# pyranha-labs/hypergrep

Measured on AMD Instinct MI355X. Metric: GiB/s scanned (256 patterns, 32 GiB synthetic log per GPU, text resident in HBM), higher is better.
Workload: dtype u8

## Files before the change

### hypergrep_amd/build.py

```python
from __future__ import annotations

import os
import shutil
import subprocess
import sys

PKG = os.path.dirname(os.path.abspath(__file__))
REPO = os.path.dirname(PKG)
CSRC = os.path.join(PKG, "csrc")
LIB_DIR = os.path.join(PKG, "lib")
LIB = os.path.join(LIB_DIR, "libhyperscanner.so")
LIBHS_NAME = "libhs.so.5"
OBJ = os.path.join(REPO, "build", "obj")
EXTRA = os.environ.get("HG_BUILD_DEFINES", "").split()
if os.environ.get("HG_BUILD_OUT"):
    LIB = os.path.abspath(os.environ["HG_BUILD_OUT"])
    LIB_DIR = os.path.dirname(LIB)
    OBJ = LIB + ".obj"
    LIBHS_NAME = os.path.basename(LIB) + ".libhs.so.5"

HIP_SOURCES = ["hg_stream.hip", "hg_kernels.hip", "hg_always_on.hip", "hg_huge.hip", "hg_som.hip", "hg_comb.hip", "hg_invert.hip", "hg_context.hip", "hg_parts.hip", "hg_segments.hip", "hg_segctx.hip", "hg_segparts.hip", "hg_gather.hip", "hg_counts.hip", "hg_flows.hip", "hg_batch.hip", "hg_engine.hip", "hg_capi.hip", "hg_shim.hip", "hg_hsface.hip"]
CXX_SOURCES = ["hg_compile.cpp"]
HEADERS = ["hg_mem.h", "hg_db.h", "hg_core.h", "hg_post.h", "hg_engine.h", "hg_compile.h", "hg_synth.h", "hg_confirm_dev.h", "hg_sink_dev.h", "hg_tables_dev.h", "hg_som.h", "hg_comb.h", "hg_invert.h", "hg_context.h", "hg_parts.h", "hg_parts_dev.h", "hg_segments.h", "hg_segctx.h", "hg_segparts.h", "hg_gather.h", "hg_counts.h", "hg_wave_dev.h", "hg_flows.h", "hg_flow_rules.h", "hg_batch.h", "hg_batch_launch.h"]


def _hipcc() -> str:
    for cand in (shutil.which("hipcc"), "/opt/rocm/bin/hipcc"):
        if cand and os.path.exists(cand):
            return cand
    raise RuntimeError("hipcc not found: the native library can only be built with the ROCm toolchain")


def _stale(target: str, deps: list[str]) -> bool:
    if not os.path.exists(target):
        return True
    t = os.path.getmtime(target)
    return any(os.path.getmtime(d) > t for d in deps if os.path.exists(d))

# ... 120 lines not shown
```

### hypergrep_amd/csrc/hg_engine.h

```cpp
#pragma once
#include <hip/hip_runtime.h>

#include <memory>
#include <string>
#include <vector>

#include "../../include/hypergrep_amd.h"
#include "hg_compile.h"
#include "hg_core.h"
#include "hg_invert.h"
#include "hg_context.h"
#include "hg_segments.h"
#include "hg_segctx.h"
#include "hg_parts.h"
#include "hg_segparts.h"
#include "hg_gather.h"
#include "hg_counts.h"
#include "hg_mem.h"
#include "hg_post.h"

#ifndef HG_STREAM_WG_WAVES
#define HG_STREAM_WG_WAVES 8
#endif
constexpr uint32_t HG_STREAM_WG_WAVES_DEFAULT = HG_STREAM_WG_WAVES;

constexpr uint32_t HG_CONFIRM_SPLIT = 4;
constexpr uint32_t HG_DEFER_SHARDS = 64;

struct HgDeferred {
  uint64_t pos;
  uint32_t pattern;
  uint32_t rank;
};
enum { HG_ST_MINLEN_KEPT = 16, HG_ST_FIN_TOTAL = 24, HG_ST_SELECTED = 28, HG_ST_FINAL = 32, HG_ST_WORDS = 36, HG_ST_ZERO_WORDS = 32,
       HG_ST_BLOCK_DONE = 40 };
enum { HG_CNT_CANDS = 0, HG_CNT_HITS = 1, HG_CNT_CAND_NEED = 2, HG_CNT_HIT_NEED = 3, HG_CNT_DEFER_NEED = 4,
       HG_CNT_HITS_WRAPPED = 5,
       HG_CNT_JOIN_TILES = 6,
       HG_CNT_WORDS = 8,
       HG_CNT_CURSOR0 = 64,
       HG_CNT_CURSORS = 64,
       HG_ST_ALLOC_WORDS = 128 };
constexpr uint32_t HG_STREAM_GRAB = 2 * HG_STREAM_WG_WAVES_DEFAULT;

constexpr uint32_t HG_FIN_MAX_BUCKETS = 1u << 22;
constexpr uint32_t HG_FIN_BUCKET_CAP = 4096;
constexpr uint32_t HG_FIN_MEDIUM_CAP = 512;

#ifndef HG_CONFIRM_THREADS
// ... 229 lines not shown
  template <typename T>
  using DevBuf = hgmem::Buf<T, hgmem::Space::Dev>;
  int device_;
  std::vector<uint32_t> ids_host_;
  hipEvent_t ev_[2] = {nullptr, nullptr};
  DevBuf<uint32_t> ids_{"counts ids", 0}, seg_lines_{"counts seg lines", 0}, seg_reports_{"counts seg reports", 0};
  DevBuf<unsigned long long> totals_{"counts totals", 0};
};

struct HgEngineKnobs {
  uint64_t fin_target = 48;
  bool no_bucket_finalize = false;
  uint64_t chunk_tiles = 0;
  uint32_t max_chunks = 0;
  std::vector<double> chunk_weights;
  long stream_wgs_per_cu = 0;
  long joiner = -1;
  bool joiner_ahead = false;
  bool no_early_finalize = false;
  uint32_t confirm_mode_mask = 0x1F;
  long confirm_blocks_per_cu = 0;
  uint64_t hit_limit = 0;
  uint64_t cand_limit = 0;
  bool verbose = false;
  static HgEngineKnobs from_env();
};

class HgScanner {
 public:
  static int create(std::shared_ptr<const HgDb> db, int device, HgScanner **out, std::string *err);
// ... 81 lines not shown
  uint64_t chunk_limit_tiles_ = 0;
  uint32_t defer_spread_boost_ = 1;
  bool hit_direct_ = false;
  HgTileSum *d_sums_ = nullptr;
  HgTileBase *d_bases_ = nullptr, *d_block_base_ = nullptr, *d_final_ = nullptr;
  HgTileElem *d_agg_ = nullptr;
  HgCand *d_cands_ = nullptr;
  HgDeferred *d_deferred_ = nullptr;
  uint32_t *d_defer_count_ = nullptr;
  HgHit *d_hits_raw_ = nullptr, *d_hits_out_ = nullptr;
  HgHitAux *d_aux_raw_ = nullptr, *d_aux_out_ = nullptr;
  HgHit *d_acc_hits_ = nullptr;
  HgHitAux *d_acc_aux_ = nullptr;
  uint64_t acc_cap_ = 0;
  bool side_bound_ = false;
  uint64_t *d_key_a_ = nullptr, *d_key_b_ = nullptr;
  uint32_t *d_perm_a_ = nullptr, *d_perm_b_ = nullptr;
  uint8_t *d_keep_ = nullptr;
  uint32_t *d_counters_ = nullptr, *d_selected_ = nullptr, *d_seg_count_ = nullptr;
  uint32_t max_segs_ = 0;
  uint32_t *d_pflags_ = nullptr;
  void *d_temp_ = nullptr;
  size_t temp_bytes_ = 0;
  uint32_t *h_counters_ = nullptr;
  HgTileBase *h_final_ = nullptr;
  hipEvent_t ev_[4] = {nullptr, nullptr, nullptr, nullptr};
  static constexpr int kMaxChunks = 64;
  hipStream_t side_stream_ = nullptr;
  hipEvent_t ev_tile_done_ = nullptr;
  hipEvent_t ev_fin_early_ = nullptr;
  hipEvent_t ev_k1_begin_[kMaxChunks] = {}, ev_k1_end_[kMaxChunks] = {}, ev_side_done_[kMaxChunks] = {};
  uint32_t *d_fin_fill_ = nullptr, *d_fin_kept_ = nullptr, *d_fin_total_ = nullptr, *d_fin_big_ = nullptr;
  bool fin_fallback_ = false;
  uint32_t fin_alloc_ = 0;
  uint32_t fin_epoch_ = 0;
  FinInfo fin_info_{};
  uint64_t fin_expect_hits_ = 0;
  void *d_huge_claim_ = nullptr;
  uint64_t huge_claim_slots_ = 0;
  uint32_t *d_from_ = nullptr;
  uint64_t from_cap_ = 0;
  uint32_t som_max_nw_ = 0;
  uint32_t *d_min_lengths_ = nullptr;
  HgHit *d_minlen_hits_ = nullptr;
  HgHitAux *d_minlen_aux_ = nullptr;
  uint64_t minlen_cap_ = 0;
  uint32_t minlen_max_nw_ = 0;
  HgComb *d_combs_ = nullptr;
  uint32_t *d_comb_words_ = nullptr, *d_comb_feed_ = nullptr;
// ... 57 lines not shown
```

### hypergrep_amd/csrc/hg_engine.hip

```cpp
#include <algorithm>
#include <array>
#include <cstdio>
#include <cstdlib>
#include <cstring>
#include <memory>

#include "hg_engine.h"
#include "hg_mem.h"

#include <rocprim/rocprim.hpp>

bool hg_launch_stream(const HgStreamArgs &a, uint32_t grid, hipStream_t stream);
bool hg_launch_stream_join(const HgStreamArgs &a, uint32_t grid, hipStream_t stream);
int hg_stream_blocks_per_cu(uint32_t filter_log2, uint32_t filter_wide, uint32_t dense);
__global__ void hg_tile_reduce_kernel(const HgTileSum *sums, uint64_t tile_begin, uint64_t tile_end, uint64_t bs1, HgTileElem *agg);
__global__ void hg_tile_spine_kernel(const HgTileElem *agg, uint32_t nblocks, uint64_t bs1, HgTileBase *block_base, HgTileBase *state);
__global__ void hg_tile_apply_kernel(const HgTileSum *sums, uint64_t tile_begin, uint64_t tile_end, uint64_t bs1, const HgTileBase *block_base,
                                     HgTileBase *bases);
__global__ void hg_tile_inner_kernel(const uint8_t *text, HgTileSum *sums, uint64_t tile_begin, uint64_t tile_end, uint64_t bs1);
__global__ void hg_verify_kernel(HgConfirmArgs a);
__global__ void hg_confirm_fast_kernel(HgConfirmArgs a, uint32_t blocks_per_mode);
__global__ void hg_confirm_generic_kernel(HgConfirmArgs a);
__global__ void hg_always_on_kernel(HgConfirmArgs a, uint32_t first, uint32_t last);
__global__ void hg_always_on_fast_kernel(HgConfirmArgs a);
// ... 20 lines not shown
__global__ void hg_offset_kernel(uint32_t *idx, uint32_t n, uint32_t add);
__global__ void hg_key_packed_kernel(const HgHit *hits, const HgHitAux *aux, const HgPattern *patterns, uint32_t n, uint32_t id_bits, uint32_t to_bits,
                                     uint64_t *key, uint32_t *idx);
__global__ void hg_keep_kernel(const HgHit *hits, const HgHitAux *aux, const uint32_t *perm, const HgPattern *patterns, uint32_t n, uint8_t *keep);
__global__ void hg_scatter_kernel(const HgHit *hits, const HgHitAux *aux, const uint32_t *perm, const uint8_t *keep, const uint32_t *pos, uint32_t n,
                                  HgHit *oh, HgHitAux *oa, uint32_t *count);

size_t hg_huge_lds_bytes(uint32_t nw_max, uint32_t stage_cap);
bool hg_launch_confirm_huge(const HgConfirmArgs &a, uint32_t grid, uint32_t nw_max, uint32_t stage_cap, void *claim, uint32_t claim_mask, hipStream_t stream);
bool hg_launch_always_on_huge(const HgConfirmArgs &a, uint32_t grid, uint32_t nw_max, uint32_t stage_cap, uint32_t first, uint32_t last, hipStream_t stream);
bool hg_launch_block_huge(const HgConfirmArgs &a, uint32_t grid, uint32_t nw_max, uint32_t stage_cap, const uint32_t *pattern_flags, hipStream_t stream);

namespace {
constexpr int TS_BLOCK_TILES = 1024;
constexpr int STREAM_WG_WAVES = HG_STREAM_WG_WAVES;

template <typename T>
hipError_t upload(void **dst, const std::vector<T> &src, const char *name) {
  size_t bytes = std::max<size_t>(src.size() * sizeof(T), 16);
  hipError_t e = hgmem::dev_alloc(dst, bytes, name);
  if (e != hipSuccess) return e;
  if (!src.empty()) e = hipMemcpy(*dst, src.data(), src.size() * sizeof(T), hipMemcpyHostToDevice);
  return e;
}
template <typename T>
hipError_t realloc_dev(T *&ptr, size_t count, const char *name) {
  hgmem::dev_free(ptr, name);
  ptr = nullptr;
  return hgmem::dev_alloc(&ptr, std::max<size_t>(count * sizeof(T), 16), name);
}
// ... 15 lines not shown
    return env ? std::strtoull(env, nullptr, 10) : dflt;
  };
  k.fin_target = std::max<uint64_t>(4, num("HG_FIN_TARGET", 48));
  k.no_bucket_finalize = std::getenv("HG_NO_BUCKET_FINALIZE") != nullptr;
  k.chunk_tiles = num("HG_CHUNK_TILES", 0);
  k.max_chunks = static_cast<uint32_t>(std::min<uint64_t>(num("HG_MAX_CHUNKS", 0), 1u << 20));
  if (const char *env = std::getenv("HG_CHUNK_WEIGHTS")) {
    for (const char *q = env; *q;) {
      char *e = nullptr;
      const double v = std::strtod(q, &e);
      if (e == q) break;
      if (v > 0) k.chunk_weights.push_back(v);
      q = *e ? e + 1 : e;
    }
  }
  k.stream_wgs_per_cu = static_cast<long>(num("HG_STREAM_WGS_PER_CU", 0));
  if (const char *env = std::getenv("HG_JOINER")) k.joiner = std::max(0l, std::min(2l, std::strtol(env, nullptr, 10)));
  k.joiner_ahead = std::getenv("HG_JOINER_AHEAD") != nullptr;
  k.no_early_finalize = std::getenv("HG_NO_EARLY_FINALIZE") != nullptr;
#ifdef HG_PROFILE_CONFIRM
  if (const char *env = std::getenv("HG_DEBUG_CONFIRM_MODES")) k.confirm_mode_mask = static_cast<uint32_t>(std::strtoul(env, nullptr, 0));
#endif
  k.confirm_blocks_per_cu = static_cast<long>(std::min<uint64_t>(num("HG_CONFIRM_BLOCKS_PER_CU", 0), 16));
  k.hit_limit = num("HG_HIT_LIMIT", 0);
  k.cand_limit = num("HG_CAND_LIMIT", 0);
  k.verbose = std::getenv("HG_VERBOSE") != nullptr;
  return k;
}

bool HgScanner::fail(hipError_t e, const char *what) {
// ... 107 lines not shown
                  d_key_a_, d_key_b_, d_perm_a_, d_perm_b_, d_keep_, d_counters_, d_temp_, d_seg_count_, d_pflags_, d_deferred_, d_defer_count_, d_seg_count2_, d_cands2_, d_disc_, d_bucket2_, d_windows2_, d_groups_, d_acc_hits_, d_acc_aux_, d_huge_claim_, d_wtab_, d_from_, d_fin_fill_, d_fin_kept_, d_fin_big_,
                  d_combs_, d_comb_words_, d_comb_feed_, d_comb_count_, d_comb_pos_, d_comb_hits_, d_comb_aux_, d_comb_temp_, d_bounds_,
                  d_min_lengths_, d_minlen_hits_, d_minlen_aux_, d_inv_count_, d_inv_pos_, d_inv_temp_, d_inv_hits_, d_inv_aux_,
                  d_ctx_count_, d_ctx_pos_, d_ctx_temp_, d_ctx_hits_, d_ctx_aux_,
                  d_parts_first_, d_parts_count_, d_parts_pos_, d_parts_temp_, d_parts_, d_part_pattern_,
                  d_segw_, d_seg_flag_, d_seg_temp_, d_seg_hits_, d_seg_aux_, d_seg_of_, d_seg_from_, d_pad_keep_, d_pad_pos_,
                  d_segctx_first_, d_segctx_k_, d_segctx_win_, d_segctx_of_, d_segparts_first_, d_segparts_of_};
  for (void *p : ptrs) hgmem::dev_free(p, "scanner");
  hgmem::host_free(h_counters_, "h_counters_");
  for (auto &ev : ev_)
    if (ev) (void)hipEventDestroy(ev);
  for (int i = 0; i < kMaxChunks; i++) {
    if (ev_k1_begin_[i]) (void)hipEventDestroy(ev_k1_begin_[i]);
    if (ev_k1_end_[i]) (void)hipEventDestroy(ev_k1_end_[i]);
    if (ev_side_done_[i]) (void)hipEventDestroy(ev_side_done_[i]);
  }
  if (side_stream_) (void)hipStreamDestroy(side_stream_);
  if (ev_fin_early_) (void)hipEventDestroy(ev_fin_early_);
  if (ev_tile_done_) (void)hipEventDestroy(ev_tile_done_);
}

int HgScanner::alloc_cands(uint64_t n) {
  n = std::min<uint64_t>(n, 0x7FFFFFF0u);
  HG_TRY(realloc_dev(d_cands_, n, "d_cands_"), "workspace alloc (candidates)");
  HG_TRY(realloc_dev(d_cands2_, n, "d_cands2_"), "workspace alloc (candidates)");
  uint32_t modes = 0;
  for (uint32_t m = 0; m < HG_CONFIRM_MODES; m++) modes += db_->n_confirm_mode[m] ? 1 : 0;
  HG_TRY(realloc_dev(d_deferred_, std::max<uint64_t>(modes, 1) * n, "d_deferred_"), "workspace alloc (deferred)");
  hgmem::dev_free(d_huge_claim_, "d_huge_claim_");
  d_huge_claim_ = nullptr;
  huge_claim_slots_ = 0;
  if (db_->n_confirm_mode[4]) {
// ... 26 lines not shown
    temp_bytes_ = need;
  }
  return HG_OK;
}

int HgScanner::ensure(uint64_t nbytes) {
  uint64_t ntiles = std::max<uint64_t>((nbytes + HG_TILE_BYTES - 1) / HG_TILE_BYTES, 1);
  auto re = [&](auto *&ptr, size_t count, const char *name) { return fail(realloc_dev(ptr, count, name), "workspace alloc"); };
  if (ntiles > cap_tiles_) {
    uint64_t nblocks = (ntiles + TS_BLOCK_TILES - 1) / TS_BLOCK_TILES;
    if (re(d_sums_, ntiles, "d_sums_") || re(d_bases_, ntiles + 1, "d_bases_") || re(d_agg_, nblocks, "d_agg_") || re(d_block_base_, nblocks, "d_block_base_")) return HG_ERR_HIP;
    cap_tiles_ = ntiles;
  }
  if (!d_seg_count_) {
    max_segs_ = static_cast<uint32_t>(num_cus_) * 16;
    if (re(d_seg_count_, max_segs_, "d_seg_count_") || re(d_seg_count2_, max_segs_, "d_seg_count2_") || re(d_defer_count_, HG_CONFIRM_MODES * HG_DEFER_SHARDS, "d_defer_count_")) return HG_ERR_HIP;
  }
  uint64_t want = std::max<uint64_t>(nbytes / 1024, 1u << 16);
  if (cand_cap_ < want && alloc_cands(want)) return HG_ERR_HIP;
  if (hit_cap_ < want && alloc_hits(want)) return HG_ERR_HIP;
  return HG_OK;
}

enum { HG_SPLIT = 1000, HG_GROWN = 1001 };

struct HgScanner::PassPlan {
  const uint8_t *text;
  uint64_t nbytes, bs1, ntiles;
  PassRange range;
  bool block_mode, has_anchored;
  hipStream_t stream, side;
  uint32_t id_bits, to_bits, fin_shift = 10, fin_nb = 1, fin_cap;
  bool bucketed;
  uint32_t nchunks = 1;
  bool piped, split;
  uint64_t chunk_tiles;
  std::array<uint64_t, kMaxChunks + 1> cut;
  uint32_t wgs_alone, wgs_shared, joiner_wgs, wgs = 1;
  uint32_t cand_seg_cap[2];
  HgStreamArgs sa;
  HgConfirmArgs ca;
  uint32_t fin_done, stage_blocks = 1;
  uint32_t wgs_of(uint32_t c) const { return c == 0 ? wgs_alone : wgs_shared; }
  uint32_t joiners_of(uint32_t c) const { return c >= 1 ? joiner_wgs : 0u; }
  uint32_t set_of(uint32_t c) const { return piped ? (c & 1u) : 0u; }
  uint32_t settled_buckets(uint32_t c) const {
    const uint64_t prev_end = std::min<uint64_t>(cut[c] << HG_TILE_SHIFT, nbytes);
    const uint64_t settled = prev_end > bs1 ? prev_end - bs1 : 0;
    return static_cast<uint32_t>(std::min<uint64_t>((settled > range.own_lo ? settled - range.own_lo : 0) >> fin_shift, fin_nb));
  }
};

HgScanner::PassPlan HgScanner::plan_pass(const uint8_t *text, uint64_t nbytes, uint64_t bs1, uint64_t line_base, const PassRange &range, bool block_mode,
                                         hipStream_t stream) const {
  const uint64_t tile_lo = range.tile_lo, tile_hi = range.tile_hi, ntiles = tile_hi - tile_lo;
  PassPlan p{text, nbytes, bs1, ntiles, range, block_mode, db_->patterns.size() - db_->ncomb > db_->slow.size(), stream};
  const uint64_t own_end = std::min<uint64_t>(range.own_hi, nbytes), own_len = own_end > range.own_lo ? own_end - range.own_lo : 0;
// ... 29 lines not shown
  if (p.split) return p;
  for (uint32_t c = 0; c <= nchunks; c++) p.cut[c] = std::min<uint64_t>(tile_lo + static_cast<uint64_t>(c) * chunk_tiles, tile_hi);
  const std::vector<double> &w = knobs_.chunk_weights;
  if (!block_mode && w.size() >= 2 && w.size() <= static_cast<size_t>(kMaxChunks) && ntiles >= w.size() * TS_BLOCK_TILES * 2) {
    double total = 0, run = 0;
    for (double v : w) total += v;
    nchunks = static_cast<uint32_t>(w.size());
    chunk_tiles = 0;
    for (uint32_t c = 0; c < nchunks; c++) {
      run += w[c];
      uint64_t end = c + 1 == nchunks ? tile_hi : tile_lo + static_cast<uint64_t>(static_cast<double>(ntiles) * run / total) / TS_BLOCK_TILES * TS_BLOCK_TILES;
      end = std::min<uint64_t>(std::max<uint64_t>(end, p.cut[c] + TS_BLOCK_TILES), tile_hi);
      p.cut[c + 1] = end;
      chunk_tiles = std::max<uint64_t>(chunk_tiles, end - p.cut[c]);
    }
  }
  p.nchunks = nchunks;
  p.chunk_tiles = chunk_tiles;
  p.piped = nchunks > 1;
  p.side = p.piped ? side_stream_ : stream;

  if (ntiles) {
    uint32_t per_cu = p.piped ? std::max(1, stream_wgs_per_cu_ - 1) : stream_wgs_per_cu_;
    if (knobs_.stream_wgs_per_cu) {
      const long v = knobs_.stream_wgs_per_cu;
      if (v >= 1 && v <= stream_wgs_per_cu_) per_cu = static_cast<uint32_t>(v);
    }
    auto grid_for = [&](uint32_t wgs_per_cu) {
      return static_cast<uint32_t>(std::min<uint64_t>((std::min<uint64_t>(chunk_tiles, ntiles) + STREAM_WG_WAVES - 1) / STREAM_WG_WAVES,
                                                      std::min<uint64_t>(static_cast<uint64_t>(num_cus_) * wgs_per_cu, max_segs_)));
    };
    p.wgs_shared = grid_for(per_cu);
    p.wgs_alone = knobs_.stream_wgs_per_cu ? p.wgs_shared : grid_for(static_cast<uint32_t>(stream_wgs_per_cu_));
    p.joiner_wgs = (p.piped && stream_wgs_per_cu_ >= 3 && per_cu < static_cast<uint32_t>(stream_wgs_per_cu_) && chunk_limit_tiles_ == 0 && !side_bound_) ? static_cast<uint32_t>(num_cus_) : 0u;
    if (knobs_.joiner >= 0) p.joiner_wgs = p.piped ? static_cast<uint32_t>(knobs_.joiner) * static_cast<uint32_t>(num_cus_) : 0u;
// ... 51 lines not shown
int HgScanner::alloc_fin(uint32_t nb, hipStream_t stream) {
  uint32_t want = 1u << 16;
  while (want < nb) want <<= 1;
  fin_alloc_ = 0;
  HG_TRY(realloc_dev(d_fin_fill_, want, "d_fin_fill_"), "alloc finalize buckets");
  HG_TRY(realloc_dev(d_fin_kept_, want, "d_fin_kept_"), "alloc finalize buckets");
  HG_TRY(realloc_dev(d_fin_big_, 2 * static_cast<size_t>(want) + 3 * 128, "d_fin_big_"), "alloc finalize buckets");
  HG_TRY(hipMemsetAsync(d_fin_big_ + 2 * static_cast<size_t>(want), 0, 3 * 128 * 4, stream), "clear scan flags");
  fin_alloc_ = want;
  return HG_OK;
}

int HgScanner::launch_fin(const PassPlan &p, hipStream_t s, uint32_t lo, uint32_t hi, bool beside_stream) {
  if (hi <= lo) return HG_OK;
  const uint32_t nbk = hi - lo, cu = static_cast<uint32_t>(num_cus_), fin_cap = p.fin_cap, id_bits = p.id_bits, to_bits = p.to_bits;
  HG_TRY(hipMemsetAsync(d_fin_total_ + 2, 0, 8, s), "memset work list");
  hipLaunchKernelGGL(hg_fin_sort_small_kernel, dim3(std::min<uint32_t>((nbk + 3) / 4, cu * 8)), dim3(256), 0, s, d_hits_raw_, d_perm_a_, d_fin_fill_, lo, hi, fin_cap, id_bits, to_bits,
                     d_fin_kept_, d_fin_big_, d_fin_total_ + 2, fin_alloc_);
  hipLaunchKernelGGL((hg_fin_sort_big_kernel<HG_FIN_MEDIUM_CAP, true>), dim3(std::min<uint32_t>(nbk, cu * 4)), dim3(256), 0, s, d_hits_raw_, d_perm_a_, d_fin_fill_, d_fin_big_, d_fin_total_ + 2,
                     fin_cap, id_bits, to_bits, d_fin_kept_, d_selected_ + 1, static_cast<uint64_t *>(nullptr), static_cast<uint32_t *>(nullptr));
  const uint32_t big_blocks = std::min<uint32_t>(std::min<uint32_t>(nbk, 64u), hit_cap_ / HG_FIN_BUCKET_CAP);
  if (big_blocks)
    hipLaunchKernelGGL((hg_fin_sort_big_kernel<HG_FIN_BUCKET_CAP, false>), dim3(big_blocks), dim3(256), 0, s, d_hits_raw_, d_perm_a_, d_fin_fill_, d_fin_big_ + fin_alloc_,
                       d_fin_total_ + 3, fin_cap, id_bits, to_bits, d_fin_kept_, d_selected_ + 1, d_key_a_, d_perm_b_);
  const uint32_t scan_blocks = std::max<uint32_t>(1, std::min<uint32_t>(128, (nbk + 8191) / 8192));
  fin_info_.scan_blocks = std::max(fin_info_.scan_blocks, scan_blocks);
  uint32_t *part = d_fin_big_ + 2 * static_cast<size_t>(fin_alloc_);
  const uint32_t epoch = ++fin_epoch_ ? fin_epoch_ : ++fin_epoch_;
  if (beside_stream) hipLaunchKernelGGL(hg_fin_scan_kernel<512u>, dim3(scan_blocks), dim3(512), 0, s, d_fin_kept_, lo, hi, d_fin_total_, d_fin_fill_, fin_cap, part, epoch);
  else hipLaunchKernelGGL(hg_fin_scan_kernel<1024u>, dim3(scan_blocks), dim3(1024), 0, s, d_fin_kept_, lo, hi, d_fin_total_, d_fin_fill_, fin_cap, part, epoch);
  hipLaunchKernelGGL(hg_fin_gather_kernel, dim3(std::min<uint32_t>((nbk + 3) / 4, cu * 8)), dim3(256), 0, s, d_hits_raw_, d_aux_raw_, d_perm_a_, d_fin_kept_, d_fin_total_, lo, hi, fin_cap,
                     d_hits_out_, d_aux_out_);
  HG_TRY(hipGetLastError(), "finalize launch");
  return HG_OK;
}

int HgScanner::copy_fin_fill(uint32_t *dst, uint32_t max, uint32_t *n) {
  *n = 0;
  if (fin_info_.path != 1u || !d_fin_fill_ || !dst) return HG_OK;
// ... 28 lines not shown
  HG_TRY(hipEventRecord(p.piped ? ev_k1_begin_[c] : ev_[1], p.stream), "event");
  if (joiners_c && knobs_.joiner_ahead)
    if (int rc = launch_joiner(p.stream)) return rc;
  if (!hg_launch_stream(sa, wgs_c, p.stream)) return error(HG_ERR_ARG, "no stream kernel for this database's filter size / mode");
  HG_TRY(hipGetLastError(), "hg_stream_kernel launch");
  HG_TRY(hipEventRecord(p.piped ? ev_k1_end_[c] : ev_[2], p.stream), "event");
  if (p.piped && p.bucketed && joiners_c && c + 1 == p.nchunks && !knobs_.no_early_finalize) {
    const uint32_t lim = p.settled_buckets(c);
    if (lim > p.fin_done) {
      if (int rc = launch_fin(p, p.side, p.fin_done, lim, true)) return rc;
      fin_info_.early_buckets += lim - p.fin_done;
      fin_info_.early_beside_stream += lim - p.fin_done;
      p.fin_done = lim;
    }
  }
  if (joiners_c && !knobs_.joiner_ahead)
    if (int rc = launch_joiner(p.side)) return rc;
  if (p.piped) HG_TRY(hipStreamWaitEvent(p.side, ev_k1_end_[c], 0), "stream wait");
  return HG_OK;
}

int HgScanner::launch_side(PassPlan &p, uint32_t c) {
  const uint64_t t0 = p.cut[c], t1 = p.cut[c + 1];
  const uint32_t segs_c = p.wgs_of(c) + p.joiners_of(c);
  const hipStream_t side = p.side;
  HgConfirmArgs ca = p.ca;
  ca.tile_begin = t0;
  ca.tile_end = t1;
  uint32_t *seg_count = p.set_of(c) ? d_seg_count2_ : d_seg_count_;
  ca.cands = p.set_of(c) ? d_cands2_ : d_cands_;
  ca.seg_count = seg_count;
  ca.cand_seg_cap = p.cand_seg_cap[c ? 1 : 0];
// ... 1 lines not shown
  ca.join_seg_cap = ca.cand_seg_cap / 4;
  uint32_t confirm_blocks = 1, always_blocks = 1;
  if (p.block_mode) {
    HG_TRY(hipMemsetAsync(d_pflags_, 0, db_->patterns.size() * 4, side), "memset pattern flags");
    if (p.has_anchored) hipLaunchKernelGGL(hg_block_mark_kernel, dim3(segs_c), dim3(256), 0, side, ca, d_pflags_);
    always_blocks = std::max<uint32_t>(static_cast<uint32_t>((db_->patterns.size() + 255) / 256), std::min<uint32_t>(db_->nhuge, 1024u));
    ca.hit_seg_cap = hit_cap_ / always_blocks;
    hipLaunchKernelGGL(hg_block_scan_kernel, dim3(static_cast<uint32_t>((db_->patterns.size() + 255) / 256)), dim3(256), 0, side, ca, d_pflags_);
    if (db_->nhuge && !hg_launch_block_huge(ca, std::min<uint32_t>(db_->nhuge, 1024u), db_->huge_max_nw, db_->huge_stage_words, d_pflags_, side)) return huge_lds_error();
    HG_TRY(hipGetLastError(), "block-mode launch");
    p.stage_blocks = std::max(confirm_blocks, always_blocks);
    return HG_OK;
  }
  const uint64_t span = t1 - t0;
  const uint32_t nblocks = static_cast<uint32_t>((span + TS_BLOCK_TILES - 1) / TS_BLOCK_TILES);
  if (p.bs1 < HG_TILE_BYTES) {
    uint32_t blocks = static_cast<uint32_t>(std::min<uint64_t>((span + 255) / 256, 4096));
    hipLaunchKernelGGL(hg_tile_inner_kernel, dim3(blocks), dim3(256), 0, side, p.text, d_sums_, t0, t1, p.bs1);
  }
  hipLaunchKernelGGL(hg_tile_reduce_kernel, dim3(nblocks), dim3(256), 0, side, d_sums_, t0, t1, p.bs1, d_agg_);
  hipLaunchKernelGGL(hg_tile_spine_kernel, dim3(1), dim3(256), 0, side, d_agg_, nblocks, p.bs1, d_block_base_, d_final_);
  hipLaunchKernelGGL(hg_tile_apply_kernel, dim3(nblocks), dim3(256), 0, side, d_sums_, t0, t1, p.bs1, d_block_base_, d_bases_);
  HG_TRY(hipGetLastError(), "tile scan launch");
  if (p.piped && c + 1 == p.nchunks) HG_TRY(hipEventRecord(ev_tile_done_, side), "event");
  if (p.has_anchored) {
    const uint32_t verify_blocks = segs_c * HG_CONFIRM_SPLIT;
    uint32_t fast_modes = 0;
    const uint32_t mode_mask = knobs_.confirm_mode_mask;
    for (uint32_t m = 0; m < 3; m++) fast_modes += (db_->n_confirm_mode[m] && ((mode_mask >> m) & 1u)) ? 1 : 0;
    uint32_t per_cu = c + 1 == p.nchunks ? 6 : 3;
    if (knobs_.confirm_blocks_per_cu) per_cu = static_cast<uint32_t>(knobs_.confirm_blocks_per_cu);
    const uint32_t mode_blocks = std::max<uint32_t>(HG_DEFER_SHARDS, static_cast<uint32_t>(num_cus_) * per_cu * (256 / HG_CONFIRM_THREADS));
    const uint32_t huge_blocks = db_->n_confirm_mode[4] ? std::max<uint32_t>(HG_DEFER_SHARDS, static_cast<uint32_t>(num_cus_) * static_cast<uint32_t>(std::max<size_t>(1, std::min<size_t>(8, (160u << 10) / std::max<size_t>(hg_huge_lds_bytes(db_->huge_max_nw, db_->huge_stage_words), 1))))) : 0u;
    confirm_blocks = std::max(std::max(mode_blocks * std::max(fast_modes, 1u), verify_blocks), huge_blocks);
    ca.hit_seg_cap = hit_cap_ / confirm_blocks;
    if (c > 0) HG_TRY(hipMemsetAsync(d_defer_count_, 0, HG_CONFIRM_MODES * HG_DEFER_SHARDS * 4, side), "memset deferred counts");
    if (ca.mode_present[1] || ca.mode_present[2]) hipLaunchKernelGGL(hg_verify_kernel, dim3(verify_blocks), dim3(256), 0, side, ca);
    else hipLaunchKernelGGL(hg_verify_lean_kernel, dim3(verify_blocks), dim3(256), 0, side, ca);
    const bool literal_only_set = ca.mode_present[0] && !ca.mode_present[1] && !ca.mode_present[2];
    if (literal_only_set) {
      hipLaunchKernelGGL(hg_confirm_literal_kernel, dim3(mode_blocks), dim3(256), 0, side, ca);
    } else if (fast_modes) {
      hipLaunchKernelGGL(hg_confirm_fast_kernel, dim3(mode_blocks * fast_modes), dim3(HG_CONFIRM_THREADS), 0, side, ca, mode_blocks);
    }
    if (db_->n_confirm_mode[3]) hipLaunchKernelGGL(hg_confirm_generic_kernel, dim3(mode_blocks), dim3(256), 0, side, ca);
    if (huge_blocks && ((mode_mask >> 4) & 1u)) {
      HG_TRY(hipMemsetAsync(d_huge_claim_, 0, huge_claim_slots_ * 8, side), "memset claim table");
      if (!hg_launch_confirm_huge(ca, huge_blocks, db_->huge_max_nw, db_->huge_stage_words, d_huge_claim_, static_cast<uint32_t>(huge_claim_slots_ - 1), side)) return huge_lds_error();
    }
    HG_TRY(hipGetLastError(), "confirm launch");
  }
  if (!db_->slow.empty()) {
    always_blocks = static_cast<uint32_t>(std::min<uint64_t>((span + 3) / 4, static_cast<uint64_t>(num_cus_) * 8));
// ... 740 lines not shown
  if (const char *why = hg_parts_refusal(db_->nhuge, db_->ncomb, db_->nquiet, db_->n_ext != 0)) return error(HG_ERR_ARG, why);
  if (int rc = scan_packed(d_text, nbytes, buffer_size, stream, params, false, out, seg)) return rc;
  return segparts_pass(stream, *out, parts, sp);
}

int HgScanner::run_once(const uint8_t *text, uint64_t nbytes, uint64_t bs1, uint64_t line_base, const PassRange &range, bool block_mode, hipStream_t stream,
                        HgScanOutput *out) {
  if (range.tile_hi > range.tile_lo && stream_wgs_per_cu_ == 0) stream_wgs_per_cu_ = hg_stream_blocks_per_cu(db_->filter_log2, db_->filter_wide, db_->dense);
  PassPlan p = plan_pass(text, nbytes, bs1, line_base, range, block_mode, stream);
  HG_TRY(hipEventRecord(ev_[0], stream), "event");
  if (p.ntiles && !fin_fallback_ && p.fin_nb > fin_alloc_)
    if (int rc = alloc_fin(p.fin_nb, stream)) return rc;
  p.bucketed = p.bucketed && d_fin_fill_;
  p.ca.bucket_cap = p.bucketed ? p.fin_cap : 0u;
  p.ca.bucket_fill = d_fin_fill_;
  fin_info_ = FinInfo{p.bucketed ? 1u : 0u, p.fin_shift, p.fin_nb, p.fin_cap, p.id_bits, p.to_bits, 0, 0, 0};
  hipLaunchKernelGGL(hg_reset_kernel, dim3(std::max<uint32_t>(1, std::min<uint32_t>((p.fin_nb + 255) / 256, 256))), dim3(256), 0, stream, d_counters_, static_cast<uint32_t>(HG_ST_ZERO_WORDS), d_final_,
                     range.cs0, range.piece0, d_fin_fill_, p.bucketed ? p.fin_nb : 0u, d_defer_count_, static_cast<uint32_t>(HG_CONFIRM_MODES * HG_DEFER_SHARDS));
  HG_TRY(hipGetLastError(), "reset launch");
  if (p.split) return HG_SPLIT;
  out->stream_launches = p.ntiles ? p.nchunks : 0;
  if (p.ntiles) {
    if (p.piped && !ev_side_done_[0])
      for (int i = 0; i < kMaxChunks; i++) {
        HG_TRY(hipEventCreate(&ev_k1_begin_[i]), "hipEventCreate");
        HG_TRY(hipEventCreate(&ev_k1_end_[i]), "hipEventCreate");
        HG_TRY(hipEventCreate(&ev_side_done_[i]), "hipEventCreate");
      }
    if (p.piped) {
      HG_TRY(hipEventRecord(ev_side_done_[kMaxChunks - 1], stream), "event");
      HG_TRY(hipStreamWaitEvent(p.side, ev_side_done_[kMaxChunks - 1], 0), "stream wait");
    }
    for (uint32_t c = 0; c < p.nchunks; c++) {
      if (p.piped && c >= 2) HG_TRY(hipStreamWaitEvent(stream, ev_side_done_[c - 2], 0), "stream wait");
      if (int rc = launch_stream(p, c, out)) return rc;
      if (int rc = launch_side(p, c)) return rc;
      if (p.bucketed && c + 1 == p.nchunks)
        if (int rc = finalize_last(p, c)) return rc;
      if (p.piped) HG_TRY(hipEventRecord(ev_side_done_[c], p.side), "event");
    }
    if (p.piped) HG_TRY(hipStreamWaitEvent(stream, ev_side_done_[p.nchunks - 1], 0), "stream wait");
  } else {
    HG_TRY(hipEventRecord(ev_[1], stream), "event");
    HG_TRY(hipEventRecord(ev_[2], stream), "event");
  }
  HG_TRY(hipMemcpyAsync(h_counters_, d_counters_, HG_ST_WORDS * 4, hipMemcpyDeviceToHost, stream), "copy state");
  if (p.bucketed) HG_TRY(hipEventRecord(ev_[3], stream), "event");
  HG_TRY(hipStreamSynchronize(stream), "stream sync (scan kernels)");
  if (p.piped) {
    uint32_t late = 0;
    for (uint32_t c = 0; c < p.nchunks; c++) {
      float ms = 0;
      (void)hipEventElapsedTime(&ms, ev_k1_begin_[c], ev_k1_end_[c]);
      out->ms_stream += ms;
      if (c >= 1 && hipEventElapsedTime(&ms, ev_k1_end_[c], ev_side_done_[c - 1]) == hipSuccess && ms > 0) late++;
    }
    side_bound_ = late * 2 > p.nchunks - 1;
  }

  out->joiner_tiles = h_counters_[HG_CNT_JOIN_TILES];
  const uint64_t n_raw = p.bucketed ? h_counters_[HG_ST_FIN_TOTAL + 1] : h_counters_[HG_CNT_HITS];
  if (int rc = regrow(p, n_raw)) return rc;
  fin_expect_hits_ = n_raw;
  const uint64_t n_pieces = block_mode ? 1 : !range.last ? 0 : h_final_->L - line_base + (nbytes > h_final_->cs ? hg_pieces(nbytes - h_final_->cs, bs1) : 0);
  uint32_t n = static_cast<uint32_t>(n_raw);
  const HgHit *fin_hits = d_hits_raw_;
  const HgHitAux *fin_aux = d_aux_raw_;
  if (n && d_min_lengths_) {
    if (int rc = minlen_pass(text, &n, p.stream)) return rc;
    fin_hits = d_minlen_hits_;
    fin_aux = d_minlen_aux_;
  }
// ... 320 lines not shown
```

Baseline: 5239.

## Add ratio-based chunk planning, optional tile stream, and per-chunk defer counters

Adds a planner that cuts the pipelined stream into geometrically shrinking chunks based on a measured or user-given ratio of side-pass cost to stream cost. It also adds an optional separate stream for the tile-scan kernels so they can overlap with verify. Both are off by default. What does run by default: per-chunk slices of the deferred-count buffer replace the per-chunk memset, and finalize work-list counters come from the already-zeroed state words instead of a memset per range. These default-on pieces remove a few small memset launches, while the rest adds complexity and more events.

```diff
diff --git a/hypergrep_amd/build.py b/hypergrep_amd/build.py
--- a/hypergrep_amd/build.py
+++ b/hypergrep_amd/build.py
@@ -21,7 +21,7 @@
 
 HIP_SOURCES = ["hg_stream.hip", "hg_kernels.hip", "hg_always_on.hip", "hg_huge.hip", "hg_som.hip", "hg_comb.hip", "hg_invert.hip", "hg_context.hip", "hg_parts.hip", "hg_segments.hip", "hg_segctx.hip", "hg_segparts.hip", "hg_gather.hip", "hg_counts.hip", "hg_flows.hip", "hg_batch.hip", "hg_engine.hip", "hg_capi.hip", "hg_shim.hip", "hg_hsface.hip"]
 CXX_SOURCES = ["hg_compile.cpp"]
-HEADERS = ["hg_mem.h", "hg_db.h", "hg_core.h", "hg_post.h", "hg_engine.h", "hg_compile.h", "hg_synth.h", "hg_confirm_dev.h", "hg_sink_dev.h", "hg_tables_dev.h", "hg_som.h", "hg_comb.h", "hg_invert.h", "hg_context.h", "hg_parts.h", "hg_parts_dev.h", "hg_segments.h", "hg_segctx.h", "hg_segparts.h", "hg_gather.h", "hg_counts.h", "hg_wave_dev.h", "hg_flows.h", "hg_flow_rules.h", "hg_batch.h", "hg_batch_launch.h"]
+HEADERS = ["hg_mem.h", "hg_db.h", "hg_core.h", "hg_post.h", "hg_engine.h", "hg_compile.h", "hg_synth.h", "hg_confirm_dev.h", "hg_sink_dev.h", "hg_tables_dev.h", "hg_som.h", "hg_comb.h", "hg_invert.h", "hg_context.h", "hg_parts.h", "hg_parts_dev.h", "hg_segments.h", "hg_segctx.h", "hg_segparts.h", "hg_gather.h", "hg_counts.h", "hg_wave_dev.h", "hg_flows.h", "hg_flow_rules.h", "hg_batch.h", "hg_batch_launch.h", "hg_plan.h"]
 
 
 def _hipcc() -> str:
diff --git a/hypergrep_amd/csrc/hg_engine.h b/hypergrep_amd/csrc/hg_engine.h
--- a/hypergrep_amd/csrc/hg_engine.h
+++ b/hypergrep_amd/csrc/hg_engine.h
@@ -17,6 +17,7 @@
 #include "hg_gather.h"
 #include "hg_counts.h"
 #include "hg_mem.h"
+#include "hg_plan.h"
 #include "hg_post.h"
 
 #ifndef HG_STREAM_WG_WAVES
@@ -32,7 +33,7 @@
   uint32_t pattern;
   uint32_t rank;
 };
-enum { HG_ST_MINLEN_KEPT = 16, HG_ST_FIN_TOTAL = 24, HG_ST_SELECTED = 28, HG_ST_FINAL = 32, HG_ST_WORDS = 36, HG_ST_ZERO_WORDS = 32,
+enum { HG_ST_FIN_LISTS = 8, HG_ST_FIN_LIST_PAIRS = 3, HG_ST_MINLEN_KEPT = 16, HG_ST_FIN_TOTAL = 24, HG_ST_SELECTED = 28, HG_ST_FINAL = 32, HG_ST_WORDS = 36, HG_ST_ZERO_WORDS = 32,
        HG_ST_BLOCK_DONE = 40 };
 enum { HG_CNT_CANDS = 0, HG_CNT_HITS = 1, HG_CNT_CAND_NEED = 2, HG_CNT_HIT_NEED = 3, HG_CNT_DEFER_NEED = 4,
        HG_CNT_HITS_WRAPPED = 5,
@@ -292,6 +293,9 @@
   uint64_t chunk_tiles = 0;
   uint32_t max_chunks = 0;
   std::vector<double> chunk_weights;
+  double chunk_ratio = 0;
+  bool chunk_ratio_auto = false;
+  long tile_stream = -1;
   long stream_wgs_per_cu = 0;
   long joiner = -1;
   bool joiner_ahead = false;
@@ -403,6 +407,7 @@
   HgHitAux *d_acc_aux_ = nullptr;
   uint64_t acc_cap_ = 0;
   bool side_bound_ = false;
+  double plan_rho_[2] = {0, 0};
   uint64_t *d_key_a_ = nullptr, *d_key_b_ = nullptr;
   uint32_t *d_perm_a_ = nullptr, *d_perm_b_ = nullptr;
   uint8_t *d_keep_ = nullptr;
@@ -416,12 +421,16 @@
   hipEvent_t ev_[4] = {nullptr, nullptr, nullptr, nullptr};
   static constexpr int kMaxChunks = 64;
   hipStream_t side_stream_ = nullptr;
+  hipStream_t tile_stream_ = nullptr;
+  hipEvent_t ev_tiles_[kMaxChunks] = {};
+  hipEvent_t ev_join_done_[kMaxChunks] = {};
   hipEvent_t ev_tile_done_ = nullptr;
   hipEvent_t ev_fin_early_ = nullptr;
   hipEvent_t ev_k1_begin_[kMaxChunks] = {}, ev_k1_end_[kMaxChunks] = {}, ev_side_done_[kMaxChunks] = {};
   uint32_t *d_fin_fill_ = nullptr, *d_fin_kept_ = nullptr, *d_fin_total_ = nullptr, *d_fin_big_ = nullptr;
   bool fin_fallback_ = false;
   uint32_t fin_alloc_ = 0;
+  uint32_t fin_ranges_ = 0;
   uint32_t fin_epoch_ = 0;
   FinInfo fin_info_{};
   uint64_t fin_expect_hits_ = 0;
diff --git a/hypergrep_amd/csrc/hg_engine.hip b/hypergrep_amd/csrc/hg_engine.hip
--- a/hypergrep_amd/csrc/hg_engine.hip
+++ b/hypergrep_amd/csrc/hg_engine.hip
@@ -58,6 +58,10 @@
 namespace {
 constexpr int TS_BLOCK_TILES = 1024;
 constexpr int STREAM_WG_WAVES = HG_STREAM_WG_WAVES;
+constexpr uint32_t kDeferCounts = HG_CONFIRM_MODES * HG_DEFER_SHARDS;
+constexpr bool kPlanByMeasuredRatio = false;
+constexpr double kPlanRatioMargin = 1.17;
+constexpr bool kTileStream = false;
 
 template <typename T>
 hipError_t upload(void **dst, const std::vector<T> &src, const char *name) {
@@ -103,6 +107,11 @@
       q = *e ? e + 1 : e;
     }
   }
+  if (const char *env = std::getenv("HG_CHUNK_RATIO")) {
+    k.chunk_ratio_auto = std::strcmp(env, "auto") == 0;
+    if (!k.chunk_ratio_auto) k.chunk_ratio = std::max(0.0, std::strtod(env, nullptr));
+  }
+  if (const char *env = std::getenv("HG_TILE_STREAM")) k.tile_stream = std::strtol(env, nullptr, 10) != 0;
   k.stream_wgs_per_cu = static_cast<long>(num("HG_STREAM_WGS_PER_CU", 0));
   if (const char *env = std::getenv("HG_JOINER")) k.joiner = std::max(0l, std::min(2l, std::strtol(env, nullptr, 10)));
   k.joiner_ahead = std::getenv("HG_JOINER_AHEAD") != nullptr;
@@ -240,8 +249,11 @@
     if (ev_k1_begin_[i]) (void)hipEventDestroy(ev_k1_begin_[i]);
     if (ev_k1_end_[i]) (void)hipEventDestroy(ev_k1_end_[i]);
     if (ev_side_done_[i]) (void)hipEventDestroy(ev_side_done_[i]);
+    if (ev_tiles_[i]) (void)hipEventDestroy(ev_tiles_[i]);
+    if (ev_join_done_[i]) (void)hipEventDestroy(ev_join_done_[i]);
   }
   if (side_stream_) (void)hipStreamDestroy(side_stream_);
+  if (tile_stream_) (void)hipStreamDestroy(tile_stream_);
   if (ev_fin_early_) (void)hipEventDestroy(ev_fin_early_);
   if (ev_tile_done_) (void)hipEventDestroy(ev_tile_done_);
 }
@@ -298,7 +310,7 @@
   }
   if (!d_seg_count_) {
     max_segs_ = static_cast<uint32_t>(num_cus_) * 16;
-    if (re(d_seg_count_, max_segs_, "d_seg_count_") || re(d_seg_count2_, max_segs_, "d_seg_count2_") || re(d_defer_count_, HG_CONFIRM_MODES * HG_DEFER_SHARDS, "d_defer_count_")) return HG_ERR_HIP;
+    if (re(d_seg_count_, max_segs_, "d_seg_count_") || re(d_seg_count2_, max_segs_, "d_seg_count2_") || re(d_defer_count_, static_cast<size_t>(kMaxChunks) * kDeferCounts, "d_defer_count_")) return HG_ERR_HIP;
   }
   uint64_t want = std::max<uint64_t>(nbytes / 1024, 1u << 16);
   if (cand_cap_ < want && alloc_cands(want)) return HG_ERR_HIP;
@@ -325,6 +337,9 @@
   HgStreamArgs sa;
   HgConfirmArgs ca;
   uint32_t fin_done, stage_blocks = 1;
+  hipStream_t tiles;
+  bool own_tiles;
+  double rho = 1;
   uint32_t wgs_of(uint32_t c) const { return c == 0 ? wgs_alone : wgs_shared; }
   uint32_t joiners_of(uint32_t c) const { return c >= 1 ? joiner_wgs : 0u; }
   uint32_t set_of(uint32_t c) const { return piped ? (c & 1u) : 0u; }
@@ -384,11 +399,18 @@
       p.cut[c + 1] = end;
       chunk_tiles = std::max<uint64_t>(chunk_tiles, end - p.cut[c]);
     }
+  } else if (!block_mode && nchunks > 1 && !chunk_limit_tiles_) {
+    const double measured = std::max(plan_rho_[0], plan_rho_[1]);
+    if (knobs_.chunk_ratio > 0) p.rho = hg_plan_clamp(knobs_.chunk_ratio);
+    else if (measured > 0 && (knobs_.chunk_ratio_auto || (kPlanByMeasuredRatio && !knobs_.chunk_tiles && !side_bound_))) p.rho = hg_plan_clamp(measured * kPlanRatioMargin);
+    if (p.rho < HG_PLAN_RHO_MAX) chunk_tiles = hg_plan_cuts(tile_lo, tile_hi, nchunks, p.rho, TS_BLOCK_TILES, p.cut.data());
   }
   p.nchunks = nchunks;
   p.chunk_tiles = chunk_tiles;
   p.piped = nchunks > 1;
   p.side = p.piped ? side_stream_ : stream;
+  p.own_tiles = p.piped && (knobs_.tile_stream < 0 ? kTileStream : knobs_.tile_stream != 0);
+  p.tiles = p.side;
 
   if (ntiles) {
     uint32_t per_cu = p.piped ? std::max(1, stream_wgs_per_cu_ - 1) : stream_wgs_per_cu_;
@@ -470,15 +492,17 @@
 int HgScanner::launch_fin(const PassPlan &p, hipStream_t s, uint32_t lo, uint32_t hi, bool beside_stream) {
   if (hi <= lo) return HG_OK;
   const uint32_t nbk = hi - lo, cu = static_cast<uint32_t>(num_cus_), fin_cap = p.fin_cap, id_bits = p.id_bits, to_bits = p.to_bits;
-  HG_TRY(hipMemsetAsync(d_fin_total_ + 2, 0, 8, s), "memset work list");
+  uint32_t *list_count = d_fin_total_ + 2;
+  if (fin_ranges_ < HG_ST_FIN_LIST_PAIRS) list_count = d_counters_ + HG_ST_FIN_LISTS + 2 * fin_ranges_++;
+  else HG_TRY(hipMemsetAsync(list_count, 0, 8, s), "memset work list");
   hipLaunchKernelGGL(hg_fin_sort_small_kernel, dim3(std::min<uint32_t>((nbk + 3) / 4, cu * 8)), dim3(256), 0, s, d_hits_raw_, d_perm_a_, d_fin_fill_, lo, hi, fin_cap, id_bits, to_bits,
-                     d_fin_kept_, d_fin_big_, d_fin_total_ + 2, fin_alloc_);
-  hipLaunchKernelGGL((hg_fin_sort_big_kernel<HG_FIN_MEDIUM_CAP, true>), dim3(std::min<uint32_t>(nbk, cu * 4)), dim3(256), 0, s, d_hits_raw_, d_perm_a_, d_fin_fill_, d_fin_big_, d_fin_total_ + 2,
+                     d_fin_kept_, d_fin_big_, list_count, fin_alloc_);
+  hipLaunchKernelGGL((hg_fin_sort_big_kernel<HG_FIN_MEDIUM_CAP, true>), dim3(std::min<uint32_t>(nbk, cu * 4)), dim3(256), 0, s, d_hits_raw_, d_perm_a_, d_fin_fill_, d_fin_big_, list_count,
                      fin_cap, id_bits, to_bits, d_fin_kept_, d_selected_ + 1, static_cast<uint64_t *>(nullptr), static_cast<uint32_t *>(nullptr));
   const uint32_t big_blocks = std::min<uint32_t>(std::min<uint32_t>(nbk, 64u), hit_cap_ / HG_FIN_BUCKET_CAP);
   if (big_blocks)
     hipLaunchKernelGGL((hg_fin_sort_big_kernel<HG_FIN_BUCKET_CAP, false>), dim3(big_blocks), dim3(256), 0, s, d_hits_raw_, d_perm_a_, d_fin_fill_, d_fin_big_ + fin_alloc_,
-                       d_fin_total_ + 3, fin_cap, id_bits, to_bits, d_fin_kept_, d_selected_ + 1, d_key_a_, d_perm_b_);
+                       list_count + 1, fin_cap, id_bits, to_bits, d_fin_kept_, d_selected_ + 1, d_key_a_, d_perm_b_);
   const uint32_t scan_blocks = std::max<uint32_t>(1, std::min<uint32_t>(128, (nbk + 8191) / 8192));
   fin_info_.scan_blocks = std::max(fin_info_.scan_blocks, scan_blocks);
   uint32_t *part = d_fin_big_ + 2 * static_cast<size_t>(fin_alloc_);
@@ -537,8 +561,10 @@
       p.fin_done = lim;
     }
   }
-  if (joiners_c && !knobs_.joiner_ahead)
+  if (joiners_c && !knobs_.joiner_ahead) {
     if (int rc = launch_joiner(p.side)) return rc;
+    if (p.own_tiles) HG_TRY(hipEventRecord(ev_join_done_[c], p.side), "event");
+  }
   if (p.piped) HG_TRY(hipStreamWaitEvent(p.side, ev_k1_end_[c], 0), "stream wait");
   return HG_OK;
 }
@@ -570,15 +596,29 @@
   }
   const uint64_t span = t1 - t0;
   const uint32_t nblocks = static_cast<uint32_t>((span + TS_BLOCK_TILES - 1) / TS_BLOCK_TILES);
+  const hipStream_t tiles = p.tiles;
+  const bool own_stream = tiles != side;
+  if (own_stream) {
+    HG_TRY(hipStreamWaitEvent(tiles, ev_k1_end_[c], 0), "stream wait");
+    if (p.joiners_of(c) && !knobs_.joiner_ahead) HG_TRY(hipStreamWaitEvent(tiles, ev_join_done_[c], 0), "stream wait");
+  }
   if (p.bs1 < HG_TILE_BYTES) {
     uint32_t blocks = static_cast<uint32_t>(std::min<uint64_t>((span + 255) / 256, 4096));
-    hipLaunchKernelGGL(hg_tile_inner_kernel, dim3(blocks), dim3(256), 0, side, p.text, d_sums_, t0, t1, p.bs1);
-  }
-  hipLaunchKernelGGL(hg_tile_reduce_kernel, dim3(nblocks), dim3(256), 0, side, d_sums_, t0, t1, p.bs1, d_agg_);
-  hipLaunchKernelGGL(hg_tile_spine_kernel, dim3(1), dim3(256), 0, side, d_agg_, nblocks, p.bs1, d_block_base_, d_final_);
-  hipLaunchKernelGGL(hg_tile_apply_kernel, dim3(nblocks), dim3(256), 0, side, d_sums_, t0, t1, p.bs1, d_block_base_, d_bases_);
+    hipLaunchKernelGGL(hg_tile_inner_kernel, dim3(blocks), dim3(256), 0, tiles, p.text, d_sums_, t0, t1, p.bs1);
+  }
+  hipLaunchKernelGGL(hg_tile_reduce_kernel, dim3(nblocks), dim3(256), 0, tiles, d_sums_, t0, t1, p.bs1, d_agg_);
+  hipLaunchKernelGGL(hg_tile_spine_kernel, dim3(1), dim3(256), 0, tiles, d_agg_, nblocks, p.bs1, d_block_base_, d_final_);
+  hipLaunchKernelGGL(hg_tile_apply_kernel, dim3(nblocks), dim3(256), 0, tiles, d_sums_, t0, t1, p.bs1, d_block_base_, d_bases_);
   HG_TRY(hipGetLastError(), "tile scan launch");
-  if (p.piped && c + 1 == p.nchunks) HG_TRY(hipEventRecord(ev_tile_done_, side), "event");
+  if (own_stream) HG_TRY(hipEventRecord(ev_tiles_[c], tiles), "event");
+  if (p.piped && c + 1 == p.nchunks) HG_TRY(hipEventRecord(ev_tile_done_, tiles), "event");
+  bool bases_awaited = !own_stream;
+  auto await_bases = [&]() -> bool {
+    if (bases_awaited) return false;
+    bases_awaited = true;
+    return fail(hipStreamWaitEvent(side, ev_tiles_[c], 0), "stream wait");
+  };
+  if (!p.has_anchored && await_bases()) return HG_ERR_HIP;
   if (p.has_anchored) {
     const uint32_t verify_blocks = segs_c * HG_CONFIRM_SPLIT;
     uint32_t fast_modes = 0;
@@ -590,9 +630,10 @@
     const uint32_t huge_blocks = db_->n_confirm_mode[4] ? std::max<uint32_t>(HG_DEFER_SHARDS, static_cast<uint32_t>(num_cus_) * static_cast<uint32_t>(std::max<size_t>(1, std::min<size_t>(8, (160u << 10) / std::max<size_t>(hg_huge_lds_bytes(db_->huge_max_nw, db_->huge_stage_words), 1))))) : 0u;
     confirm_blocks = std::max(std::max(mode_blocks * std::max(fast_modes, 1u), verify_blocks), huge_blocks);
     ca.hit_seg_cap = hit_cap_ / confirm_blocks;
-    if (c > 0) HG_TRY(hipMemsetAsync(d_defer_count_, 0, HG_CONFIRM_MODES * HG_DEFER_SHARDS * 4, side), "memset deferred counts");
+    ca.defer_count = d_defer_count_ + static_cast<size_t>(c) * kDeferCounts;
     if (ca.mode_present[1] || ca.mode_present[2]) hipLaunchKernelGGL(hg_verify_kernel, dim3(verify_blocks), dim3(256), 0, side, ca);
     else hipLaunchKernelGGL(hg_verify_lean_kernel, dim3(verify_blocks), dim3(256), 0, side, ca);
+    if (await_bases()) return HG_ERR_HIP;
     const bool literal_only_set = ca.mode_present[0] && !ca.mode_present[1] && !ca.mode_present[2];
     if (literal_only_set) {
       hipLaunchKernelGGL(hg_confirm_literal_kernel, dim3(mode_blocks), dim3(256), 0, side, ca);
@@ -1363,9 +1404,10 @@
   p.bucketed = p.bucketed && d_fin_fill_;
   p.ca.bucket_cap = p.bucketed ? p.fin_cap : 0u;
   p.ca.bucket_fill = d_fin_fill_;
+  fin_ranges_ = 0;
   fin_info_ = FinInfo{p.bucketed ? 1u : 0u, p.fin_shift, p.fin_nb, p.fin_cap, p.id_bits, p.to_bits, 0, 0, 0};
   hipLaunchKernelGGL(hg_reset_kernel, dim3(std::max<uint32_t>(1, std::min<uint32_t>((p.fin_nb + 255) / 256, 256))), dim3(256), 0, stream, d_counters_, static_cast<uint32_t>(HG_ST_ZERO_WORDS), d_final_,
-                     range.cs0, range.piece0, d_fin_fill_, p.bucketed ? p.fin_nb : 0u, d_defer_count_, static_cast<uint32_t>(HG_CONFIRM_MODES * HG_DEFER_SHARDS));
+                     range.cs0, range.piece0, d_fin_fill_, p.bucketed ? p.fin_nb : 0u, d_defer_count_, p.nchunks * kDeferCounts);
   HG_TRY(hipGetLastError(), "reset launch");
   if (p.split) return HG_SPLIT;
   out->stream_launches = p.ntiles ? p.nchunks : 0;
@@ -1376,6 +1418,16 @@
         HG_TRY(hipEventCreate(&ev_k1_end_[i]), "hipEventCreate");
         HG_TRY(hipEventCreate(&ev_side_done_[i]), "hipEventCreate");
       }
+    if (p.own_tiles) {
+      if (!tile_stream_) {
+        HG_TRY(hipStreamCreateWithFlags(&tile_stream_, hipStreamNonBlocking), "hipStreamCreate");
+        for (int i = 0; i < kMaxChunks; i++) {
+          HG_TRY(hipEventCreateWithFlags(&ev_tiles_[i], hipEventDisableTiming), "hipEventCreate");
+          HG_TRY(hipEventCreateWithFlags(&ev_join_done_[i], hipEventDisableTiming), "hipEventCreate");
+        }
+      }
+      p.tiles = tile_stream_;
+    }
     if (p.piped) {
       HG_TRY(hipEventRecord(ev_side_done_[kMaxChunks - 1], stream), "event");
       HG_TRY(hipStreamWaitEvent(p.side, ev_side_done_[kMaxChunks - 1], 0), "stream wait");
@@ -1405,6 +1457,22 @@
       if (c >= 1 && hipEventElapsedTime(&ms, ev_k1_end_[c], ev_side_done_[c - 1]) == hipSuccess && ms > 0) late++;
     }
     side_bound_ = late * 2 > p.nchunks - 1;
+    double begin[kMaxChunks], end[kMaxChunks], done[kMaxChunks];
+    bool timed = kPlanByMeasuredRatio || knobs_.chunk_ratio_auto || knobs_.verbose;
+    for (uint32_t c = 0; timed && c < p.nchunks; c++) {
+      float b = 0, e = 0, d = 0;
+      timed = timed && hipEventElapsedTime(&b, ev_k1_begin_[0], ev_k1_begin_[c]) == hipSuccess && hipEventElapsedTime(&e, ev_k1_begin_[0], ev_k1_end_[c]) == hipSuccess &&
+              hipEventElapsedTime(&d, ev_k1_begin_[0], ev_side_done_[c]) == hipSuccess;
+      begin[c] = b, end[c] = e, done[c] = d;
+    }
+    const double rho = timed ? hg_plan_measure(p.cut.data(), p.nchunks, begin, end, done) : 0;
+    if (rho > 0) plan_rho_[1] = plan_rho_[0], plan_rho_[0] = rho;
+    if (knobs_.verbose) {
+      std::fprintf(stderr, "hypergrep_amd: pass of %u chunks cut by ratio %.3f, measured %.3f, side-bound %d;", p.nchunks, p.rho, rho, side_bound_ ? 1 : 0);
+      for (uint32_t c = 0; timed && c < p.nchunks; c++)
+        std::fprintf(stderr, " [%llu tiles: stream %.3f ms, side passes done %.3f ms after it]", static_cast<unsigned long long>(p.cut[c + 1] - p.cut[c]), end[c] - begin[c], done[c] - end[c]);
+      std::fprintf(stderr, "\n");
+    }
   }
 
   out->joiner_tiles = h_counters_[HG_CNT_JOIN_TILES];
diff --git a/hypergrep_amd/csrc/hg_plan.h b/hypergrep_amd/csrc/hg_plan.h
--- /dev/null
+++ b/hypergrep_amd/csrc/hg_plan.h
@@ -0,0 +1,58 @@
+#pragma once
+#include <algorithm>
+#include <cmath>
+#include <cstdint>
+
+constexpr double HG_PLAN_RHO_MIN = 0.5, HG_PLAN_RHO_MAX = 1.0;
+inline double hg_plan_clamp(double rho) { return !(rho > HG_PLAN_RHO_MIN) ? HG_PLAN_RHO_MIN : rho < HG_PLAN_RHO_MAX ? rho : HG_PLAN_RHO_MAX; }
+
+inline uint64_t hg_plan_equal_chunk(uint64_t ntiles, uint32_t n, uint64_t block) {
+  return ((ntiles + n - 1) / n + block - 1) / block * block;
+}
+
+inline uint64_t hg_plan_cuts(uint64_t tile_lo, uint64_t tile_hi, uint32_t n, double rho, uint64_t block, uint64_t *cut) {
+  const uint64_t ntiles = tile_hi - tile_lo, nblocks = (ntiles + block - 1) / block;
+  rho = hg_plan_clamp(rho);
+  if (rho >= HG_PLAN_RHO_MAX || nblocks < n || n < 2) {
+    const uint64_t chunk = std::max<uint64_t>(hg_plan_equal_chunk(ntiles, n, block), block);
+    for (uint32_t c = 0; c <= n; c++) cut[c] = std::min<uint64_t>(tile_lo + static_cast<uint64_t>(c) * chunk, tile_hi);
+    return std::min(chunk, ntiles);
+  }
+  auto next = [rho](uint64_t b) { return std::max<uint64_t>(1, static_cast<uint64_t>(std::ceil(rho * static_cast<double>(b) - 1e-9))); };
+  auto total = [&](uint64_t b0) {
+    uint64_t sum = 0, b = b0;
+    for (uint32_t c = 0; c < n; c++, b = next(b)) sum += b;
+    return sum;
+  };
+  uint64_t lo = 1, hi = nblocks;
+  while (lo < hi) {
+    const uint64_t mid = lo + (hi - lo + 1) / 2;
+    if (total(mid) <= nblocks) lo = mid;
+    else hi = mid - 1;
+  }
+  uint64_t left = nblocks - total(lo), b = lo, at = tile_lo, largest = 0;
+  cut[0] = tile_lo;
+  for (uint32_t c = 0; c < n; c++, b = next(b)) {
+    uint64_t blocks = b;
+    if (c + 2 != n && left) {
+      const uint64_t share = c + 1 == n ? left : 1;
+      blocks += share;
+      left -= share;
+    }
+    at = c + 1 == n ? tile_hi : at + blocks * block;
+    cut[c + 1] = at;
+    largest = std::max(largest, cut[c + 1] - cut[c]);
+  }
+  return largest;
+}
+
+inline double hg_plan_measure(const uint64_t *cut, uint32_t n, const double *stream_begin, const double *stream_end, const double *side_done) {
+  double rho = 0;
+  for (uint32_t c = 0; c + 1 < n; c++) {
+    const double chain = side_done[c] - std::max(stream_end[c], c ? side_done[c - 1] : stream_end[c]);
+    const double launch = stream_end[c + 1] - stream_begin[c + 1];
+    const double tiles_c = static_cast<double>(cut[c + 1] - cut[c]), tiles_n = static_cast<double>(cut[c + 2] - cut[c + 1]);
+    if (chain > 0 && launch > 0 && tiles_c > 0 && tiles_n > 0) rho = std::max(rho, (chain / tiles_c) / (launch / tiles_n));
+  }
+  return rho;
+}
```

After: 5248, median of 6. No clear change (+0.2%).
